# happierpig/flashinfer-ai

Hardware: AMD Instinct MI355X
Metric: paged_decode_hbm_bandwidth_bs64_kv8192_hd128 (higher is better)
Workload: dtype bf16; 1 GPU; C2: BatchDecodeWithPagedKVCacheWrapper bf16 GQA 32/8 head_dim=128 page_size=16 bs=64/GPU kv_len=8192, random page permutation; batch_per_gpu=64, kv_len=8192, num_qo_heads=32, num_kv_heads=8, head_dim=128, page_size=16, split_kv=True, kv_chunk_size=4096, parallelism=batch-shard x1 (no data-path collective)

## Files before the change

### flashinfer-ai_amd/csrc/decode.hip

```cpp
#include <stdlib.h>
#include <string.h>

#include <algorithm>
#include <vector>

#include "decode_kernel.h"
#include "merge_kernel.h"

namespace fi {

#define FI_DECL(DT, HD)                                                                   \
  hipError_t decode_launch_##DT##_##HD(const DecodeKernelParams& p, int gt, int rope, int grid, \
                                       hipStream_t stream);
FI_DECL(0, 64) FI_DECL(0, 128) FI_DECL(0, 256) FI_DECL(0, 512)
FI_DECL(1, 64) FI_DECL(1, 128) FI_DECL(1, 256) FI_DECL(1, 512)
FI_DECL(2, 64) FI_DECL(2, 128) FI_DECL(2, 256) FI_DECL(2, 512)
FI_DECL(3, 64) FI_DECL(3, 128) FI_DECL(3, 256) FI_DECL(3, 512)
#undef FI_DECL

typedef hipError_t (*decode_launch_fn)(const DecodeKernelParams&, int, int, int, hipStream_t);

static decode_launch_fn find_launcher(int kv_dt, int head_dim) {
#define FI_ROW(DT)                          \
  case DT:                                  \
// ... 18 lines not shown
      return nullptr;
  }
#undef FI_ROW
}

static bool decode_mfma16() {
  static const bool on = [] {
    const char* e = getenv("FI_DECODE_MFMA16");
    return !e || atoi(e) != 0;
  }();
  return on;
}

static int decode_waves_per_cu(int kv_dtype, bool batch) {
  const bool fp8 = kv_dtype == FI_DTYPE_FP8_E4M3 || kv_dtype == FI_DTYPE_FP8_E5M2;
  return (batch && !fp8) ? 4 : 8;
}

static int tokens_per_load(int kv_dt, int head_dim) {
  const int vec = 16 / (int)dtype_size(kv_dt);
  return 64 / (head_dim / vec);
}

static int ilog2_exact(int x) {
  if (x <= 0 || (x & (x - 1))) return -1;
  int l = 0;
  while ((1 << l) < x) ++l;
  return l;
}

hipError_t decode_mfma_launch(const DecodeKernelParams& p, int q_dtype, int kv_dtype, int head_dim, int rope, int grid,
                              hipStream_t stream);
hipError_t decode_mfma16_launch(const DecodeKernelParams& p, int q_dtype, int kv_dtype, int head_dim, int rope,
                                int grid, hipStream_t stream);

constexpr int kMfmaMinGroup = 5;
constexpr int kMfmaMinGroupFp8 = 3;

enum class DecodeKernel { VALU, MFMA32, MFMA16 };

struct DecodeChoice {
  DecodeKernel kind;
  int head_tiles;
  int gt;
};

static DecodeChoice choose_decode(int group, int q_dt, int kv_dt, int head_dim, int page_size, bool rope,
                                  bool plain_logits, bool strides_fit_31_bits) {
  DecodeChoice c;
  c.gt = group <= 1 ? 1 : group == 2 ? 2 : 4;
  const bool fp8 = kv_dt == FI_DTYPE_FP8_E4M3 || kv_dt == FI_DTYPE_FP8_E5M2;
  const bool mfma = (q_dt == FI_DTYPE_F16 || q_dt == FI_DTYPE_BF16) && (kv_dt == q_dt || fp8) &&
                    (head_dim == 64 || head_dim == 128) && strides_fit_31_bits;
  if (decode_mfma16()) {
    c.kind = !(mfma && (plain_logits || group <= 16)) ? DecodeKernel::VALU
             : group <= 16                            ? DecodeKernel::MFMA16
                                                      : DecodeKernel::MFMA32;
  } else {
    const bool small_pages = ilog2_exact(page_size) < 0 || page_size < tokens_per_load(kv_dt, head_dim);
    const int min_group = (rope || small_pages) ? 1 : fp8 ? kMfmaMinGroupFp8 : kMfmaMinGroup;
    c.kind = mfma && plain_logits && group >= min_group ? DecodeKernel::MFMA32 : DecodeKernel::VALU;
  }
  c.head_tiles = c.kind == DecodeKernel::VALU ? ceil_div(group, c.gt) : ceil_div(group, 32);
  return c;
}

static int launch_decode(const DecodeKernelParams& kp, const DecodeChoice& c, int q_dt, int kv_dt, int head_dim,
                         bool rope, int merge_n, int merge_rows, hipStream_t stream) {
  if (kp.num_items > 0) {
    const int grid = ceil_div(kp.num_items, kDecodeWaves);
    if (c.kind == DecodeKernel::MFMA16)
      FI_HIP_CALL(decode_mfma16_launch(kp, q_dt, kv_dt, head_dim, rope, grid, stream));
    else if (c.kind == DecodeKernel::MFMA32)
      FI_HIP_CALL(decode_mfma_launch(kp, q_dt, kv_dt, head_dim, rope, grid, stream));
    else
      FI_HIP_CALL(find_launcher(kv_dt, head_dim)(kp, c.gt, rope, grid, stream));
  }
  if (kp.split_kv) {
    MergeNParams mp{kp.tmp_o, kp.tmp_lse, kp.o_indptr, kp.o, kp.lse, merge_n, merge_rows,
                    kp.num_qo_heads, head_dim, FI_DTYPE_F32, q_dt};
    FI_HIP_CALL(launch_merge_n(mp, stream));
  }
  return 0;
}

static int32_t window_pages(const int32_t* indptr_h, int i, int page_size, int window_left) {
  const int32_t np = indptr_h[i + 1] - indptr_h[i];
  if (window_left < 0 || np <= 0) return np;
  const int64_t first = std::max<int64_t>((int64_t)(np - 1) * page_size - window_left, 0) / page_size;
  return (int32_t)(np - first);
}

struct DecodeWork {
  bool split_kv;
  uint32_t pages_per_chunk;
  size_t padded;
};

static DecodeWork estimate_decode_work(const int32_t* indptr_h, int batch_size, int page_size, int window_left,
                                       uint32_t gdy, uint32_t max_grid, bool enable_cuda_graph) {
  std::vector<int32_t> num_pages(batch_size);
  uint32_t max_pages = 0;
  for (int i = 0; i < batch_size; ++i)
    max_pages = std::max<uint32_t>(max_pages, num_pages[i] = window_pages(indptr_h, i, page_size, window_left));
  if ((uint64_t)batch_size * gdy >= max_grid) return {false, std::max(max_pages, 1u), (size_t)batch_size};
// ... 31 lines not shown
  FI_REQUIRE(find_launcher(kv_dtype, head_dim) != nullptr,
             "batch_decode_plan: unsupported kv dtype %d / head_dim %d", kv_dtype, head_dim);
  for (int i = 0; i < batch_size; ++i)
    FI_REQUIRE(indptr_h[i + 1] >= indptr_h[i], "batch_decode_plan: indptr must be non-decreasing");

  const int head_tiles = choose_decode(num_qo_heads / num_kv_heads, q_dtype, kv_dtype, head_dim, page_size,
                                       false, true, true)
                             .head_tiles;
  const uint32_t gdy = (uint32_t)(num_kv_heads * head_tiles);
  const uint32_t max_grid =
      max_grid_hint > 0 ? (uint32_t)max_grid_hint
                        : (uint32_t)(fi_num_compute_units() * decode_waves_per_cu(kv_dtype, true) * (head_tiles > 1 ? 2 : 1));

  if (window_left < 0) window_left = -1;
  const auto [split_kv, pages_per_chunk, padded] =
      estimate_decode_work(indptr_h, batch_size, page_size, window_left, gdy, max_grid, enable_cuda_graph);

  OffsetAllocator ia(int_ws_bytes);
  const int64_t req_off = ia.alloc(padded * sizeof(int32_t));
  const int64_t tile_off = ia.alloc(padded * sizeof(int32_t));
  const int64_t oind_off = ia.alloc(((size_t)batch_size + 1) * sizeof(int32_t));
  const int64_t chunk_off = ia.alloc(sizeof(int32_t));
  int64_t mask_off = 0;
  if (split_kv) mask_off = ia.alloc(padded);
  FI_REQUIRE(ia.ok, "batch_decode_plan: int workspace too small (%zu bytes)", int_ws_bytes);

  char* hp = (char*)pinned_int_ws;
  int32_t* req_h = (int32_t*)(hp + req_off);
  int32_t* tile_h = (int32_t*)(hp + tile_off);
  int32_t* oind_h = (int32_t*)(hp + oind_off);
  memset(req_h, 0, padded * sizeof(int32_t));
  memset(tile_h, 0, padded * sizeof(int32_t));
  size_t w = 0;
  oind_h[0] = 0;
  for (int b = 0; b < batch_size; ++b) {
    const uint32_t np = (uint32_t)std::max(window_pages(indptr_h, b, page_size, window_left), 1);
    const uint32_t nchunks = split_kv ? ceil_div(np, pages_per_chunk) : 1u;
    for (uint32_t t = 0; t < nchunks; ++t) {
      FI_REQUIRE(w < padded, "batch_decode_plan: work list overflow");
      req_h[w] = b;
      tile_h[w] = (int32_t)t;
      ++w;
    }
    oind_h[b + 1] = oind_h[b] + (int32_t)nchunks;
  }
  *(int32_t*)(hp + chunk_off) = (int32_t)(pages_per_chunk * (uint32_t)page_size);
  if (split_kv) {
    uint8_t* mask_h = (uint8_t*)(hp + mask_off);
    for (size_t i = 0; i < padded; ++i) mask_h[i] = i < w;
  }

  int64_t v_off = 0, s_off = 0;
  if (split_kv) {
    OffsetAllocator fa(float_ws_bytes);
    v_off = fa.alloc((size_t)num_qo_heads * padded * head_dim * sizeof(float));
    s_off = fa.alloc((size_t)num_qo_heads * padded * sizeof(float));
    FI_REQUIRE(fa.ok, "batch_decode_plan: float workspace too small (%zu bytes, need %zu)",
               float_ws_bytes, (size_t)num_qo_heads * padded * (head_dim + 1) * sizeof(float));
  }

  for (int i = 0; i < FI_DECODE_PLAN_INFO_LEN; ++i) plan_info_out[i] = 0;
  plan_info_out[FI_DP_PADDED_BATCH_SIZE] = (int64_t)padded;
  plan_info_out[FI_DP_V_OFFSET] = v_off;
  plan_info_out[FI_DP_S_OFFSET] = s_off;
  plan_info_out[FI_DP_REQUEST_INDICES_OFFSET] = req_off;
  plan_info_out[FI_DP_KV_TILE_INDICES_OFFSET] = tile_off;
  plan_info_out[FI_DP_O_INDPTR_OFFSET] = oind_off;
  plan_info_out[FI_DP_BLOCK_VALID_MASK_OFFSET] = mask_off;
  plan_info_out[FI_DP_KV_CHUNK_SIZE_PTR_OFFSET] = chunk_off;
  plan_info_out[FI_DP_ENABLE_CUDA_GRAPH] = enable_cuda_graph ? 1 : 0;
  plan_info_out[FI_DP_SPLIT_KV] = split_kv ? 1 : 0;
  plan_info_out[FI_DP_KV_CHUNK_SIZE] = (int64_t)pages_per_chunk * page_size;
  plan_info_out[FI_DP_NUM_WORK] = (int64_t)w;
  plan_info_out[FI_DP_BATCH_SIZE] = batch_size;
  plan_info_out[FI_DP_INT_BYTES_USED] = (int64_t)ia.used;
  plan_info_out[FI_DP_WINDOW_LEFT] = window_left;
  plan_info_out[FI_DP_MAGIC] = FI_DECODE_PLAN_MAGIC;

  if (int_ws && ia.used)
    FI_HIP_CALL(hipMemcpyAsync(int_ws, pinned_int_ws, ia.used, hipMemcpyHostToDevice,
                               (hipStream_t)stream));
  return 0;
}

namespace fi {

template <class A>
static int check_and_fill_decode(const char* who, const A& a, int kv_dt, int head_dim, int num_kv_heads,
                                 int page_size, int64_t kv_stride_page, int64_t kv_stride_n, int64_t kv_stride_h,
                                 DecodeKernelParams& kp, DecodeChoice& choice) {
  FI_REQUIRE(a.q_dtype == FI_DTYPE_F16 || a.q_dtype == FI_DTYPE_BF16, "%s: q dtype must be f16/bf16", who);
  FI_REQUIRE(num_kv_heads > 0 && a.num_qo_heads % num_kv_heads == 0,
             "%s: num_qo_heads must be a multiple of num_kv_heads", who);
  FI_REQUIRE(find_launcher(kv_dt, head_dim), "%s: unsupported kv dtype %d / head_dim %d", who, kv_dt, head_dim);
  FI_REQUIRE(a.pos_encoding_mode != FI_POS_ALIBI || a.alibi_slopes, "%s: ALIBI needs alibi_slopes", who);
  memset(&kp, 0, sizeof(kp));
  kp.q = a.q;
  kp.o = a.o;
  kp.lse = a.lse;
  kp.alibi_slopes = a.alibi_slopes;
  kp.kv_stride_page = kv_stride_page;
  kp.kv_stride_n = kv_stride_n;
  kp.kv_stride_h = kv_stride_h;
  kp.num_qo_heads = a.num_qo_heads;
  kp.num_kv_heads = num_kv_heads;
  kp.group_size = a.num_qo_heads / num_kv_heads;
  kp.page_size = page_size;
  kp.log2_page_size = ilog2_exact(page_size);
  kp.uniform_page = kp.log2_page_size >= 0 && page_size >= tokens_per_load(kv_dt, head_dim);
  kp.page_div = FastDiv((uint32_t)page_size);
  kp.window_left = a.window_left;
  kp.q_dtype = a.q_dtype;
  kp.use_alibi = a.pos_encoding_mode == FI_POS_ALIBI;
  kp.logits_soft_cap = a.logits_soft_cap > 0.f ? a.logits_soft_cap : 0.f;
  kp.sm_scale = a.sm_scale;
  kp.rope_rcp_scale = a.rope_rcp_scale;
  kp.rope_rcp_theta = a.rope_rcp_theta;
  const bool plain_logits = a.pos_encoding_mode != FI_POS_ALIBI && !(a.logits_soft_cap > 0.f);
  choice = choose_decode(kp.group_size, a.q_dtype, kv_dt, head_dim, page_size,
                         a.pos_encoding_mode == FI_POS_ROPE_LLAMA, plain_logits,
                         kv_stride_page < (1ll << 31) && kv_stride_n < (1ll << 31));
  kp.head_tiles = choice.head_tiles;
  return 0;
}

}

extern "C" FI_API int fi_batch_decode_run(void* float_ws, size_t float_ws_bytes, void* int_ws,
                                   size_t int_ws_bytes, const int64_t* plan_info,
                                   int32_t plan_info_len, const fi_batch_decode_params_t* a,
                                   fi_stream_t stream_) {
  hipStream_t stream = (hipStream_t)stream_;
  FI_REQUIRE(plan_info && plan_info_len == FI_DECODE_PLAN_INFO_LEN &&
                 plan_info[FI_DP_MAGIC] == FI_DECODE_PLAN_MAGIC,
             "batch_decode_run: plan_info is not a decode plan (call plan() first)");
  FI_REQUIRE(a && a->q && a->o && a->kv.k_data && a->kv.v_data && a->kv.indptr &&
                 a->kv.last_page_len,
             "batch_decode_run: null tensor");
  FI_REQUIRE(int_ws, "batch_decode_run: null int workspace");
  const fi_paged_kv_t& kv = a->kv;
  FI_REQUIRE(kv.batch_size == plan_info[FI_DP_BATCH_SIZE],
             "batch_decode_run: batch size %d differs from the planned %lld", kv.batch_size,
             (long long)plan_info[FI_DP_BATCH_SIZE]);
  FI_REQUIRE(a->pos_encoding_mode >= 0 && a->pos_encoding_mode <= 2,
             "batch_decode_run: bad pos_encoding_mode %d", a->pos_encoding_mode);
  DecodeKernelParams kp;
  DecodeChoice choice;
  if (check_and_fill_decode("batch_decode_run", *a, kv.dtype, kv.head_dim, kv.num_kv_heads, kv.page_size,
                            kv.stride_page, kv.stride_n, kv.stride_h, kp, choice))
    return 1;
  const size_t esz = dtype_size(kv.dtype);
  FI_REQUIRE(((uintptr_t)a->q % 16) == 0 && (a->q_stride_n * 2) % 16 == 0 && (a->q_stride_h * 2) % 16 == 0,
             "batch_decode_run: q rows must be 16-byte aligned");
  FI_REQUIRE((kv.stride_n * esz) % 16 == 0 && (kv.stride_h * esz) % 16 == 0 &&
                 (kv.stride_page * esz) % 16 == 0 && ((uintptr_t)kv.k_data % 16) == 0 &&
                 ((uintptr_t)kv.v_data % 16) == 0,
             "batch_decode_run: kv cache rows must be 16-byte aligned");
  if (kv.batch_size == 0) return 0;

  const bool split = plan_info[FI_DP_SPLIT_KV] != 0;
  const int64_t padded = plan_info[FI_DP_PADDED_BATCH_SIZE];
  kp.k = kv.k_data;
  kp.v = kv.v_data;
  kp.indptr = kv.indptr;
  kp.indices = kv.indices;
  kp.last_page_len = kv.last_page_len;
  const char* ib = (const char*)int_ws;
  kp.request_indices = (const int32_t*)(ib + plan_info[FI_DP_REQUEST_INDICES_OFFSET]);
  kp.kv_tile_indices = (const int32_t*)(ib + plan_info[FI_DP_KV_TILE_INDICES_OFFSET]);
  kp.o_indptr = (const int32_t*)(ib + plan_info[FI_DP_O_INDPTR_OFFSET]);
  kp.block_valid_mask =
      (split && plan_info[FI_DP_ENABLE_CUDA_GRAPH])
          ? (const uint8_t*)(ib + plan_info[FI_DP_BLOCK_VALID_MASK_OFFSET])
          : nullptr;
  (void)int_ws_bytes;
  kp.q_rope_offset = a->q_rope_offset;
  kp.kv_rope_pos_offset = kv.rope_pos_offset;
  kp.q_stride_n = a->q_stride_n;
  kp.q_stride_h = a->q_stride_h;
  kp.num_items = (int32_t)(padded * kv.num_kv_heads * kp.head_tiles);
  kp.kv_chunk_size = (int32_t)plan_info[FI_DP_KV_CHUNK_SIZE];
  kp.kv_chunk_size_ptr = (const int32_t*)(ib + plan_info[FI_DP_KV_CHUNK_SIZE_PTR_OFFSET]);
  kp.split_kv = split;
  kp.plan_window_left = (int32_t)plan_info[FI_DP_WINDOW_LEFT];
  FI_REQUIRE(kp.plan_window_left < 0 || kp.plan_window_left == a->window_left,
             "batch_decode_run: window_left %d differs from the planned %d", a->window_left, kp.plan_window_left);
  if (split) {
    FI_REQUIRE(float_ws, "batch_decode_run: split-kv plan needs the float workspace");
    const size_t need = (size_t)plan_info[FI_DP_S_OFFSET] +
                        (size_t)a->num_qo_heads * padded * sizeof(float);
    FI_REQUIRE(need <= float_ws_bytes, "batch_decode_run: float workspace too small");
    kp.tmp_o = (float*)((char*)float_ws + plan_info[FI_DP_V_OFFSET]);
    kp.tmp_lse = (float*)((char*)float_ws + plan_info[FI_DP_S_OFFSET]);
  }
  kp.fast_path = kp.uniform_page && kp.indices && !kp.use_alibi && kp.logits_soft_cap == 0.f;
  return launch_decode(kp, choice, a->q_dtype, kv.dtype, kv.head_dim, a->pos_encoding_mode == FI_POS_ROPE_LLAMA,
                       0, kv.batch_size, stream);
}

extern "C" FI_API int fi_single_decode_run(const fi_single_decode_params_t* a, void* tmp, size_t tmp_bytes,
                                    fi_stream_t stream_) {
  hipStream_t stream = (hipStream_t)stream_;
  FI_REQUIRE(a && a->q && a->k && a->v && a->o, "single_decode_run: null tensor");
  FI_REQUIRE(a->kv_len >= 0, "single_decode_run: negative kv_len");
  const int vpage = 16;
  DecodeKernelParams kp;
  DecodeChoice choice;
  if (check_and_fill_decode("single_decode_run", *a, a->kv_dtype, a->head_dim, a->num_kv_heads, vpage,
                            (int64_t)vpage * a->kv_stride_n, a->kv_stride_n, a->kv_stride_h, kp, choice))
    return 1;
  const size_t esz = dtype_size(a->kv_dtype);
  FI_REQUIRE(((uintptr_t)a->q % 16) == 0 && (a->q_stride_h * 2) % 16 == 0,
             "single_decode_run: q rows must be 16-byte aligned");
  FI_REQUIRE((a->kv_stride_n * esz) % 16 == 0 && (a->kv_stride_h * esz) % 16 == 0 &&
                 ((uintptr_t)a->k % 16) == 0 && ((uintptr_t)a->v % 16) == 0,
             "single_decode_run: k/v rows must be 16-byte aligned");

  kp.k = a->k;
  kp.v = a->v;
  kp.q_stride_n = 0;
  kp.q_stride_h = a->q_stride_h;
  kp.single_kv_len = a->kv_len;
  kp.plan_window_left = -1;
  const int gdy = a->num_kv_heads * kp.head_tiles;
  const int max_grid = fi_num_compute_units() * decode_waves_per_cu(a->kv_dtype, false);
  int chunk = a->kv_len, nchunks = 1;
  if (a->kv_len > 256 && tmp) {
    const int want = std::max(1, max_grid / gdy);
    chunk = std::max(ceil_div(a->kv_len, want), 256);
    chunk = ceil_div(chunk, vpage) * vpage;
    nchunks = ceil_div(a->kv_len, chunk);
    const size_t need = (size_t)nchunks * a->num_qo_heads * (a->head_dim + 1) * sizeof(float) + 64;
    if (need > tmp_bytes || nchunks <= 1) {
      chunk = a->kv_len;
      nchunks = 1;
    }
  }
  kp.split_kv = nchunks > 1;
  kp.kv_chunk_size = chunk;
  kp.num_items = nchunks * gdy;
  if (kp.split_kv) {
    kp.tmp_o = (float*)tmp;
    size_t vbytes = (size_t)nchunks * a->num_qo_heads * a->head_dim * sizeof(float);
    vbytes = (vbytes + 15) / 16 * 16;
    kp.tmp_lse = (float*)((char*)tmp + vbytes);
  }
  return launch_decode(kp, choice, a->q_dtype, a->kv_dtype, a->head_dim, a->pos_encoding_mode == FI_POS_ROPE_LLAMA,
                       nchunks, 1, stream);
}
```

### flashinfer-ai_amd/csrc/decode_mfma16_inst.hip

```cpp
#include "decode_mfma16_kernel.h"

namespace fi {

template <int T16, int KVS, int D>
static hipError_t launch16(const DecodeKernelParams& p, int rope, int grid, hipStream_t stream) {
  const dim3 g(grid), b(kDecodeThreads);
  if (rope) {
    if (p.indices) decode_mfma16_kernel<T16, KVS, D, true, true><<<g, b, 0, stream>>>(p);
    else decode_mfma16_kernel<T16, KVS, D, false, true><<<g, b, 0, stream>>>(p);
  } else {
    if (p.indices) decode_mfma16_kernel<T16, KVS, D, true, false><<<g, b, 0, stream>>>(p);
    else decode_mfma16_kernel<T16, KVS, D, false, false><<<g, b, 0, stream>>>(p);
  }
  return hipGetLastError();
}

hipError_t decode_mfma16_launch(const DecodeKernelParams& p, int q_dtype, int kv_dtype, int head_dim, int rope,
                                int grid, hipStream_t stream) {
#define FI_CASE(T, K, D) \
  if (q_dtype == T && kv_dtype == K && head_dim == D) return launch16<T, K, D>(p, rope, grid, stream);
#define FI_ROW(T, K) FI_CASE(T, K, 64) FI_CASE(T, K, 128)
  FI_ROW(FI_DTYPE_F16, FI_DTYPE_F16)
  FI_ROW(FI_DTYPE_F16, FI_DTYPE_FP8_E4M3)
  FI_ROW(FI_DTYPE_F16, FI_DTYPE_FP8_E5M2)
  FI_ROW(FI_DTYPE_BF16, FI_DTYPE_BF16)
  FI_ROW(FI_DTYPE_BF16, FI_DTYPE_FP8_E4M3)
  FI_ROW(FI_DTYPE_BF16, FI_DTYPE_FP8_E5M2)
#undef FI_ROW
#undef FI_CASE
  return hipErrorInvalidValue;
}

}
```

### flashinfer-ai_amd/csrc/decode_mfma16_kernel.h

```cpp
#pragma once
#include "decode_kernel.h"
#include "prefill_kernel.h"

namespace fi {

template <int T16>
struct Mfma16;
template <>
struct Mfma16<FI_DTYPE_F16> {
  static __device__ __forceinline__ f32x4 mfma(MfmaType<FI_DTYPE_F16>::frag a, MfmaType<FI_DTYPE_F16>::frag b, f32x4 c) {
    return __builtin_amdgcn_mfma_f32_16x16x32_f16(a, b, c, 0, 0, 0);
  }
};
template <>
struct Mfma16<FI_DTYPE_BF16> {
  static __device__ __forceinline__ f32x4 mfma(MfmaType<FI_DTYPE_BF16>::frag a, MfmaType<FI_DTYPE_BF16>::frag b, f32x4 c) {
    return __builtin_amdgcn_mfma_f32_16x16x32_bf16(a, b, c, 0, 0, 0);
  }
};

template <bool MAX>
__device__ __forceinline__ float reduce_rows(float x) {
  const uint32_t u = __builtin_bit_cast(uint32_t, x);
  const auto r = __builtin_amdgcn_permlane16_swap(u, u, false, false);
  const uint32_t r0 = r[0], r1 = r[1];
  const float a = __builtin_bit_cast(float, r0), b = __builtin_bit_cast(float, r1);
  const float y = MAX ? fmaxf(a, b) : a + b;
  const uint32_t v = __builtin_bit_cast(uint32_t, y);
  const auto q = __builtin_amdgcn_permlane32_swap(v, v, false, false);
  const uint32_t q0 = q[0], q1 = q[1];
  const float c = __builtin_bit_cast(float, q0), d = __builtin_bit_cast(float, q1);
  return MAX ? fmaxf(c, d) : c + d;
}

template <int T16, int KVS, int D, bool PAGED, bool ROPE>
__global__ void __launch_bounds__(kDecodeThreads, (ROPE && D == 128 && KVS != T16) ? 1 : 2)
    decode_mfma16_kernel(const DecodeKernelParams p) {
  using M = MfmaType<T16>;
  using frag_t = typename M::frag;
  constexpr int kTile = 32;
  constexpr bool KV_FP8 = (KVS == FI_DTYPE_FP8_E4M3 || KVS == FI_DTYPE_FP8_E5M2);
  constexpr int KV_BYTES = KV_FP8 ? 1 : 2;
  constexpr int ROWB = D * 2;
  constexpr int CPR = D / 8;
  constexpr int GCH = D * KV_BYTES / 16;
  constexpr int RPP = 64 / GCH;
  constexpr int NPASS = kTile / RPP;
  constexpr int KSTEPS = D / 32;
  constexpr int DBLK = D / 16;
  constexpr int TILE_BYTES = kTile * ROWB;
  constexpr int NE = KV_FP8 ? 16 : 8;
  static_assert(D == 64 || D == 128, "head_dim 64 / 128");

  __shared__ __attribute__((aligned(16))) char smem[kDecodeWaves][2 * TILE_BYTES];
  __shared__ __attribute__((aligned(16))) float rope_step[ROPE ? GCH * NE * 2 : 4];

  const int lane = threadIdx.x & 63;
  const int wave = __builtin_amdgcn_readfirstlane((int)(threadIdx.x >> 6));
  int lb;
  {
    const int b = blockIdx.x, total = gridDim.x;
    const int xcd = b & 7, slot = b >> 3;
    const int qn = total >> 3, rn = total & 7;
    lb = (xcd < rn ? xcd * (qn + 1) : rn * (qn + 1) + (xcd - rn) * qn) + slot;
  }
  const int item = lb * kDecodeWaves + wave;
  if (item >= p.num_items) return;
  char* const kb = smem[wave];
  char* const vb = kb + TILE_BYTES;
  const int lc = lane & 15, lg = lane >> 4;

  const int kv_head = item % p.num_kv_heads;
  const int work = item / p.num_kv_heads;
  int req = 0, kv_tile = work;
  if (p.request_indices) {
    if (p.block_valid_mask && !p.block_valid_mask[work]) return;
    req = p.request_indices[work];
    kv_tile = p.kv_tile_indices[work];
  }
  int page_begin = 0, kv_len;
  if (p.indptr) {
    page_begin = p.indptr[req];
    const int np = p.indptr[req + 1] - page_begin;
    kv_len = np > 0 ? (np - 1) * p.page_size + p.last_page_len[req] : 0;
  } else {
    kv_len = p.single_kv_len;
  }
  int chunk_base = 0;
  if (p.plan_window_left >= 0 && p.indptr) {
    const int np = p.indptr[req + 1] - page_begin;
    chunk_base = np > 0 ? max((np - 1) * p.page_size - p.plan_window_left, 0) / p.page_size * p.page_size : 0;
  }
  const int win_start = p.window_left >= 0 ? max(0, kv_len - 1 - p.window_left) : 0;
  const int kv_chunk_size = p.kv_chunk_size_ptr ? *p.kv_chunk_size_ptr : p.kv_chunk_size;
  int chunk_start = chunk_base + (p.split_kv ? kv_tile * kv_chunk_size : 0);
  const int chunk_end = p.split_kv ? min(chunk_start + kv_chunk_size, kv_len) : kv_len;
  if (win_start > chunk_start) chunk_start += (win_start - chunk_start) / kTile * kTile;
  const int G = p.group_size;
  const int head0 = kv_head * G;
  const int head = head0 + min(lc, G - 1);

  frag_t qf[KSTEPS];
  {
    const uint16_t* qrow = (const uint16_t*)p.q + (int64_t)req * p.q_stride_n + (int64_t)head * p.q_stride_h;
#pragma unroll
    for (int ks = 0; ks < KSTEPS; ++ks)
      qf[ks] = __builtin_bit_cast(frag_t, *(const u32x4*)(qrow + 32 * ks + 8 * lg));
    if constexpr (ROPE) {
      const int q_pos = p.q_rope_offset ? p.q_rope_offset[req] : (kv_len - 1);
#pragma unroll
      for (int ks = 0; ks < KSTEPS / 2; ++ks) {
        const u32x4 lo4 = __builtin_bit_cast(u32x4, qf[ks]), hi4 = __builtin_bit_cast(u32x4, qf[ks + KSTEPS / 2]);
        u32x4 out_lo, out_hi;
#pragma unroll
        for (int w = 0; w < 4; ++w) {
          const uint32_t lo_w = lo4[w], hi_w = hi4[w];
          float ra[2], rb[2];
#pragma unroll
          for (int e = 0; e < 2; ++e) {
            const int i = 32 * ks + 8 * lg + 2 * w + e;
            const float freq = p.rope_rcp_scale * __powf(p.rope_rcp_theta, (float)(2 * i) / (float)D);
            float sn, cs;
            sincos_ool((float)q_pos * freq, &sn, &cs);
            const float a = M::to_f32((uint16_t)(lo_w >> (16 * e)));
            const float b = M::to_f32((uint16_t)(hi_w >> (16 * e)));
            ra[e] = a * cs - b * sn;
            rb[e] = b * cs + a * sn;
          }
          out_lo[w] = pack2<T16>(ra[0], ra[1]);
// ... 220 lines not shown
      for (int h = 0; h < 2; ++h)
#pragma unroll
        for (int j2 = 0; j2 < 2; ++j2) {
          const float a = s_acc[h][2 * j2], b = s_acc[h][2 * j2 + 1];
          const uint32_t pk = pack2<T16>(a, b);
          w[2 * h + j2] = pk;
          if constexpr (T16 == FI_DTYPE_BF16) {
            const float ha = __builtin_bit_cast(float, pk << 16);
            const float hb = __builtin_bit_cast(float, pk & 0xffff0000u);
            wl[2 * h + j2] = pack2<T16>(a - ha, b - hb);
          }
        }
      const frag_t pfrag = __builtin_bit_cast(frag_t, w);
#pragma unroll
      for (int db = 0; db < DBLK; ++db) {
        const char* base = vb + v_rd[db];
        const s16x4 lo = __builtin_amdgcn_ds_read_tr16_b64_v4i16((__attribute__((address_space(3))) s16x4*)(base));
        const s16x4 hi = __builtin_amdgcn_ds_read_tr16_b64_v4i16(
            (__attribute__((address_space(3))) s16x4*)(base + 16 * ROWB));
        using s16x8 = __attribute__((ext_vector_type(8))) short;
        const s16x8 a8 = {lo[0], lo[1], lo[2], lo[3], hi[0], hi[1], hi[2], hi[3]};
        o_acc[db] = Mfma16<T16>::mfma(__builtin_bit_cast(frag_t, a8), pfrag, o_acc[db]);
        if constexpr (T16 == FI_DTYPE_BF16)
          o_acc[db] = Mfma16<T16>::mfma(__builtin_bit_cast(frag_t, a8), __builtin_bit_cast(frag_t, wl), o_acc[db]);
      }
      __builtin_amdgcn_wave_barrier();
    }
  }

  l_run = reduce_rows<false>(l_run);
  const bool empty = !(l_run > 0.f);
  const float inv = empty ? 0.f : 1.0f / l_run;
  const float lse_v = empty ? FI_NEG_INF : m_run + fast_log2(l_run);
  if (lc < G) {
    const int qo_head = head0 + lc;
    const int64_t out_row = p.split_kv ? (int64_t)(p.o_indptr ? p.o_indptr[req] : 0) + kv_tile : req;
    const int64_t ob = (out_row * p.num_qo_heads + qo_head) * D;
#pragma unroll
    for (int db = 0; db < DBLK; ++db) {
      const int d0 = 16 * db + 4 * lg;
      if (p.split_kv) {
        *(f32x4*)(p.tmp_o + ob + d0) = o_acc[db] * inv;
      } else {
        const uint32_t w0 = pack2<T16>(o_acc[db][0] * inv, o_acc[db][1] * inv);
        const uint32_t w1 = pack2<T16>(o_acc[db][2] * inv, o_acc[db][3] * inv);
        *(u32x2*)((uint16_t*)p.o + ob + d0) = u32x2{w0, w1};
      }
    }
    if (lg == 0) {
      if (p.split_kv) p.tmp_lse[out_row * p.num_qo_heads + qo_head] = lse_v;
      else if (p.lse) p.lse[out_row * p.num_qo_heads + qo_head] = lse_v;
    }
  }
}

}
```

### flashinfer-ai_amd/flashinfer/_lib.py

```python
from __future__ import annotations

import ctypes as C
import os
from typing import Optional

import torch

_HERE = os.path.dirname(os.path.abspath(__file__))
_LIB_PATH = os.environ.get("FI_MI355_LIB", os.path.join(_HERE, "libfi_mi355.so"))

FI_DTYPE_F16, FI_DTYPE_BF16, FI_DTYPE_FP8_E4M3, FI_DTYPE_FP8_E5M2, FI_DTYPE_F32 = range(5)
FI_NEG_INF = -5.0e4
FI_DECODE_PLAN_INFO_LEN = 16

_TORCH2FI = {
    torch.float16: FI_DTYPE_F16,
    torch.bfloat16: FI_DTYPE_BF16,
    torch.float8_e4m3fn: FI_DTYPE_FP8_E4M3,
    torch.float8_e5m2: FI_DTYPE_FP8_E5M2,
    torch.float32: FI_DTYPE_F32,
}


def fi_dtype(dtype: torch.dtype) -> int:
    try:
        return _TORCH2FI[dtype]
    except KeyError:
        raise ValueError(f"unsupported dtype {dtype} for the MI355X kernels") from None


class PagedKV(C.Structure):
    _fields_ = [
        ("k_data", C.c_void_p),
        ("v_data", C.c_void_p),
        ("indptr", C.c_void_p),
        ("indices", C.c_void_p),
        ("last_page_len", C.c_void_p),
        ("rope_pos_offset", C.c_void_p),
        ("stride_page", C.c_int64),
        ("stride_n", C.c_int64),
        ("stride_h", C.c_int64),
        ("page_size", C.c_int32),
        ("num_kv_heads", C.c_int32),
        ("head_dim", C.c_int32),
        ("batch_size", C.c_int32),
        ("dtype", C.c_int32),
# ... 212 lines not shown
    _fields_ = [
        ("in_", C.c_void_p), ("out", C.c_void_p), ("top_k_arr", C.c_void_p), ("scalar_arr", C.c_void_p),
        ("top_k_val", C.c_int32), ("scalar_val", C.c_float),
        ("batch", C.c_int32), ("vocab", C.c_int32), ("param_len", C.c_int32),
    ]


class ChainSpeculativeParams(C.Structure):
    _fields_ = [
        ("draft_probs", C.c_void_p), ("draft_token_ids", C.c_void_p), ("target_probs", C.c_void_p),
        ("output_token_ids", C.c_void_p), ("output_accepted_token_num", C.c_void_p),
        ("output_emitted_draft_token_num", C.c_void_p),
        ("batch", C.c_int32), ("num_speculative_tokens", C.c_int32), ("vocab", C.c_int32),
        ("philox_seed", C.c_uint64), ("philox_offset", C.c_uint64),
    ]


FI_PREFILL_PLAN_INFO_LEN = 16
FI_PREFILL_PLAN_MAGIC = 0x4649505245
FI_PREFILL_QKVO_PLAN_MAGIC = 0x4649514B564F
FI_MLA_PLAN_INFO_LEN = 16
(FI_MLA_NUM_WORK, FI_MLA_GRID, FI_MLA_TOTAL_ROWS, FI_MLA_KV_CHUNK_SIZE, FI_MLA_SPLIT_KV, FI_MLA_ENABLE_CUDA_GRAPH,
 FI_MLA_NUM_HEADS, FI_MLA_BATCH_SIZE, FI_MLA_INT_BYTES_USED, FI_MLA_MERGE_INDPTR_OFFSET, FI_MLA_ITEMS_OFFSET,
 FI_MLA_NUM_ENTRIES, FI_MLA_V_OFFSET, FI_MLA_PAGE_SIZE, FI_MLA_DTYPE, FI_MLA_MAGIC) = range(16)

_lib: Optional[C.CDLL] = None

EXPORTED_SYMBOLS = [
    "fi_last_error",
    "fi_abi_version",
    "fi_num_compute_units",
    "fi_batch_decode_plan",
    "fi_batch_decode_run",
    "fi_single_decode_run",
    "fi_merge_state",
    "fi_merge_state_in_place",
    "fi_merge_states",
    "fi_variable_length_merge_states",
    "fi_batch_prefill_plan",
    "fi_batch_prefill_paged_run",
    "fi_single_prefill_run",
    "fi_batch_prefill_qkvo_run",
    "fi_single_prefill_qkvo_run",
    "fi_gemm_fp8_nt_groupwise",
    "fi_group_gemm_fp8_nt_groupwise",
    "fi_get_batch_indices_positions",
    "fi_append_paged_kv_cache",
    "fi_apply_rope_pos_ids",
    "fi_apply_rope_append_paged_kv_cache",
    "fi_rope_positions_from_indptr",
    "fi_packbits",
    "fi_segment_packbits",
    "fi_batch_mla_plan",
    "fi_batch_mla_run",
    "fi_append_paged_mla_kv_cache",
    "fi_softmax",
    "fi_sampling_from_logits",
    "fi_sampling_from_probs",
    "fi_top_k_sampling_from_probs",
    "fi_top_p_sampling_from_probs",
    "fi_min_p_sampling_from_probs",
    "fi_top_k_top_p_sampling_from_probs",
    "fi_top_p_renorm_probs",
    "fi_top_k_renorm_probs",
    "fi_top_k_mask_logits",
    "fi_chain_speculative_sampling",
]

SAMPLING_SYMBOLS = ("fi_sampling_from_logits", "fi_sampling_from_probs", "fi_top_k_sampling_from_probs",
                    "fi_top_p_sampling_from_probs", "fi_min_p_sampling_from_probs",
                    "fi_top_k_top_p_sampling_from_probs")
ROW_TRANSFORM_SYMBOLS = ("fi_softmax", "fi_top_p_renorm_probs", "fi_top_k_renorm_probs", "fi_top_k_mask_logits")


def lib() -> C.CDLL:
    global _lib
    if _lib is not None:
        return _lib
    if not os.path.exists(_LIB_PATH):
        raise RuntimeError(
            f"{_LIB_PATH} not found: build it with `make -C flashinfer-ai_amd/csrc -j8` "
            "(or python -c 'import __graft_entry__ as g; g.build()').  There is no CPU fallback."
        )
    l = C.CDLL(_LIB_PATH)
    l.fi_last_error.restype = C.c_char_p
    l.fi_abi_version.restype = C.c_int
    l.fi_num_compute_units.restype = C.c_int
    vp, i32, i64p, sz = C.c_void_p, C.c_int32, C.POINTER(C.c_int64), C.c_size_t
    l.fi_batch_decode_plan.argtypes = [vp, sz, vp, vp, sz, vp, i32, i32, i32, i32, i32, i32, i32, i32, i32, i32, i64p, vp]
    l.fi_batch_decode_run.argtypes = [vp, sz, vp, sz, i64p, i32, C.POINTER(BatchDecodeParams), vp]
    l.fi_single_decode_run.argtypes = [C.POINTER(SingleDecodeParams), vp, sz, vp]
    l.fi_merge_state.argtypes = [vp, vp, vp, vp, vp, vp, i32, i32, i32, i32, vp]
    l.fi_merge_state_in_place.argtypes = [vp, vp, vp, vp, vp, i32, i32, i32, i32, vp]
    l.fi_merge_states.argtypes = [vp, vp, vp, vp, i32, i32, i32, i32, i32, vp]
    l.fi_variable_length_merge_states.argtypes = [vp, vp, vp, vp, vp, i32, i32, i32, i32, i32, vp]
    l.fi_batch_prefill_plan.argtypes = [vp, sz, vp, vp, sz, vp, vp, vp] + [i32] * 12 + [i64p, vp]
    l.fi_batch_prefill_paged_run.argtypes = [vp, sz, vp, sz, i64p, i32, C.POINTER(BatchPrefillParams), vp]
    l.fi_single_prefill_run.argtypes = [C.POINTER(SinglePrefillParams), vp, sz, vp]
    l.fi_batch_prefill_qkvo_run.argtypes = [vp, sz, vp, sz, i64p, i32, C.POINTER(PrefillQkvoParams), vp]
    l.fi_single_prefill_qkvo_run.argtypes = [C.POINTER(PrefillQkvoParams), vp, sz, vp]
    l.fi_gemm_fp8_nt_groupwise.argtypes = [vp] * 5 + [i32] * 10 + [vp]
    l.fi_group_gemm_fp8_nt_groupwise.argtypes = [vp] * 6 + [i32] * 11 + [vp]
    l.fi_packbits.argtypes = [vp, C.c_int64, i32, vp, vp]
    l.fi_segment_packbits.argtypes = [vp, vp, vp, i32, C.c_int64, i32, vp, vp]
    l.fi_get_batch_indices_positions.argtypes = [vp, vp, i32, i32, vp, vp, vp]
    l.fi_append_paged_kv_cache.argtypes = [vp, vp, C.c_int64, C.c_int64, C.c_int64, C.c_int64, vp, vp, i32, C.POINTER(PagedKV), vp]
    l.fi_apply_rope_pos_ids.argtypes = [C.POINTER(RopeParams), vp]
    l.fi_apply_rope_append_paged_kv_cache.argtypes = [C.POINTER(RopeParams), vp, C.c_int64, C.c_int64, vp, vp, C.POINTER(PagedKV), vp]
    l.fi_rope_positions_from_indptr.argtypes = [vp, vp, i32, i32, vp, vp]
    l.fi_batch_mla_plan.argtypes = [C.POINTER(MlaPlanParams), i64p, vp]
    l.fi_batch_mla_run.argtypes = [i64p, i32, C.POINTER(MlaParams), vp]
    l.fi_append_paged_mla_kv_cache.argtypes = [C.POINTER(AppendMlaParams), vp]
    for name in SAMPLING_SYMBOLS:
        getattr(l, name).argtypes = [C.POINTER(SamplingParams), vp]
    for name in ROW_TRANSFORM_SYMBOLS:
        getattr(l, name).argtypes = [C.POINTER(RowTransformParams), vp]
    l.fi_chain_speculative_sampling.argtypes = [C.POINTER(ChainSpeculativeParams), vp]
    for name in EXPORTED_SYMBOLS:
        fn = getattr(l, name)
        if name not in ("fi_last_error",):
            fn.restype = C.c_int
    _lib = l
    return l
# ... 60 lines not shown
```

### include/fi_mi355.h

```cpp
#ifndef FI_MI355_H_
#define FI_MI355_H_

#include <stddef.h>
#include <stdint.h>

#ifdef __cplusplus
extern "C" {
#endif

#define FI_ABI_VERSION 2
#define FI_NEG_INF (-5.0e4f)

typedef void* fi_stream_t;

#if defined(FI_BUILDING_LIB)
#define FI_API __attribute__((visibility("default")))
#else
#define FI_API
#endif

enum fi_dtype {
  FI_DTYPE_F16 = 0,
  FI_DTYPE_BF16 = 1,
  FI_DTYPE_FP8_E4M3 = 2,
  FI_DTYPE_FP8_E5M2 = 3,
  FI_DTYPE_F32 = 4
};

enum fi_pos_encoding_mode { FI_POS_NONE = 0, FI_POS_ROPE_LLAMA = 1, FI_POS_ALIBI = 2 };
enum fi_mask_mode { FI_MASK_NON_CAUSAL = 0, FI_MASK_CAUSAL = 1, FI_MASK_CUSTOM = 2, FI_MASK_MULTIITEMSCORING = 3 };

FI_API const char* fi_last_error(void);
FI_API int fi_abi_version(void);
FI_API int fi_num_compute_units(void);

typedef struct fi_paged_kv {
  const void* k_data;
  const void* v_data;
  const int32_t* indptr;
  const int32_t* indices;
  const int32_t* last_page_len;
  const int32_t* rope_pos_offset;
  int64_t stride_page, stride_n, stride_h;
  int32_t page_size;
  int32_t num_kv_heads;
  int32_t head_dim;
  int32_t batch_size;
  int32_t dtype;
} fi_paged_kv_t;

#define FI_DECODE_PLAN_INFO_LEN 16
enum fi_decode_plan_slot {
  FI_DP_PADDED_BATCH_SIZE = 0,
  FI_DP_V_OFFSET = 1,
  FI_DP_S_OFFSET = 2,
  FI_DP_REQUEST_INDICES_OFFSET = 3,
  FI_DP_KV_TILE_INDICES_OFFSET = 4,
  FI_DP_O_INDPTR_OFFSET = 5,
  FI_DP_BLOCK_VALID_MASK_OFFSET = 6,
  FI_DP_KV_CHUNK_SIZE_PTR_OFFSET = 7,
  FI_DP_ENABLE_CUDA_GRAPH = 8,
  FI_DP_SPLIT_KV = 9,
  FI_DP_KV_CHUNK_SIZE = 10,
  FI_DP_NUM_WORK = 11,
  FI_DP_BATCH_SIZE = 12,
  FI_DP_INT_BYTES_USED = 13,
  FI_DP_WINDOW_LEFT = 14,
  FI_DP_MAGIC = 15
};
#define FI_DECODE_PLAN_MAGIC 0x4649444543ll

FI_API int fi_batch_decode_plan(void* float_ws, size_t float_ws_bytes, void* int_ws, void* pinned_int_ws,
                         size_t int_ws_bytes, const int32_t* indptr_h, int32_t batch_size,
                         int32_t num_qo_heads, int32_t num_kv_heads, int32_t page_size,
                         int32_t enable_cuda_graph, int32_t head_dim, int32_t q_dtype,
                         int32_t kv_dtype, int32_t max_grid_hint, int32_t window_left,
                         int64_t* plan_info_out, fi_stream_t stream);

typedef struct fi_batch_decode_params {
  const void* q;
  int64_t q_stride_n, q_stride_h;
  fi_paged_kv_t kv;
  void* o;
  float* lse;
  const float* alibi_slopes;
  const int32_t* q_rope_offset;
  int32_t num_qo_heads;
  int32_t q_dtype;
  int32_t pos_encoding_mode;
  int32_t window_left;
  float logits_soft_cap;
  float sm_scale;
  float rope_rcp_scale;
  float rope_rcp_theta;
} fi_batch_decode_params_t;

FI_API int fi_batch_decode_run(void* float_ws, size_t float_ws_bytes, void* int_ws, size_t int_ws_bytes,
                        const int64_t* plan_info, int32_t plan_info_len,
                        const fi_batch_decode_params_t* params, fi_stream_t stream);

typedef struct fi_single_decode_params {
  const void* q;
  int64_t q_stride_h;
  const void* k;
  const void* v;
  int64_t kv_stride_n, kv_stride_h;
  void* o;
  float* lse;
  const float* alibi_slopes;
  int32_t kv_len, num_qo_heads, num_kv_heads, head_dim;
  int32_t q_dtype, kv_dtype;
  int32_t pos_encoding_mode;
  int32_t window_left;
  float logits_soft_cap, sm_scale, rope_rcp_scale, rope_rcp_theta;
} fi_single_decode_params_t;

FI_API int fi_single_decode_run(const fi_single_decode_params_t* params, void* tmp, size_t tmp_bytes,
                         fi_stream_t stream);

FI_API int fi_merge_state(const void* v_a, const float* s_a, const void* v_b, const float* s_b,
                   void* v_merged, float* s_merged, int32_t seq_len, int32_t num_heads,
                   int32_t head_dim, int32_t dtype, fi_stream_t stream);
FI_API int fi_merge_state_in_place(void* v, float* s, const void* v_other, const float* s_other,
                            const uint8_t* mask, int32_t seq_len, int32_t num_heads,
                            int32_t head_dim, int32_t dtype, fi_stream_t stream);
FI_API int fi_merge_states(const void* v, const float* s, void* v_merged, float* s_merged,
                    int32_t num_index_sets, int32_t seq_len, int32_t num_heads, int32_t head_dim,
                    int32_t dtype, fi_stream_t stream);
FI_API int fi_variable_length_merge_states(const void* v, const float* s, const int32_t* indptr,
                                    void* v_merged, float* s_merged, int32_t seq_len,
                                    int32_t num_heads, int32_t head_dim, int32_t in_dtype,
                                    int32_t out_dtype, fi_stream_t stream);
// ... 293 lines not shown
```

Measured before the change: 6651 GB/s.

## Fold split-KV chunks into one workgroup and merge in LDS, dropping merge kernel

When a paged MFMA16 split-KV decode has at most four chunks per request, the waves of one workgroup each process a chunk of the same request and KV head. The partial outputs and LSEs go through shared memory and are combined by the chunk-0 wave, which writes the final output directly. This removes the separate merge launch and the round trip of the fp32 tmp_o/tmp_lse buffers through HBM. In exchange, fewer KV heads are handled per workgroup, a workgroup-wide barrier is added, and the plan info gains a max_chunks slot, which changes the ABI length.

```diff
diff --git a/flashinfer-ai_amd/csrc/decode.hip b/flashinfer-ai_amd/csrc/decode.hip
--- a/flashinfer-ai_amd/csrc/decode.hip
+++ b/flashinfer-ai_amd/csrc/decode.hip
@@ -74,7 +74,7 @@
 hipError_t decode_mfma_launch(const DecodeKernelParams& p, int q_dtype, int kv_dtype, int head_dim, int rope, int grid,
                               hipStream_t stream);
 hipError_t decode_mfma16_launch(const DecodeKernelParams& p, int q_dtype, int kv_dtype, int head_dim, int rope,
-                                int grid, hipStream_t stream);
+                                int nc, int grid, hipStream_t stream);
 
 constexpr int kMfmaMinGroup = 5;
 constexpr int kMfmaMinGroupFp8 = 3;
@@ -107,12 +107,24 @@
   return c;
 }
 
+static int decode_fold_chunks(const DecodeChoice& c, bool split_kv, bool graph_plan, int64_t max_chunks, bool rope,
+                              bool paged) {
+  if (!split_kv || graph_plan || c.kind != DecodeKernel::MFMA16 || rope || !paged) return 0;
+  if (max_chunks < 1 || max_chunks > 4) return 0;
+  return max_chunks <= 2 ? 2 : 4;
+}
+
 static int launch_decode(const DecodeKernelParams& kp, const DecodeChoice& c, int q_dt, int kv_dt, int head_dim,
-                         bool rope, int merge_n, int merge_rows, hipStream_t stream) {
+                         bool rope, int merge_n, int merge_rows, int fold_nc, hipStream_t stream) {
+  if (fold_nc) {
+    const int grid = merge_rows * ceil_div(kp.num_kv_heads, kDecodeWaves / fold_nc);
+    FI_HIP_CALL(decode_mfma16_launch(kp, q_dt, kv_dt, head_dim, rope, fold_nc, grid, stream));
+    return 0;
+  }
   if (kp.num_items > 0) {
     const int grid = ceil_div(kp.num_items, kDecodeWaves);
     if (c.kind == DecodeKernel::MFMA16)
-      FI_HIP_CALL(decode_mfma16_launch(kp, q_dt, kv_dt, head_dim, rope, grid, stream));
+      FI_HIP_CALL(decode_mfma16_launch(kp, q_dt, kv_dt, head_dim, rope, 0, grid, stream));
     else if (c.kind == DecodeKernel::MFMA32)
       FI_HIP_CALL(decode_mfma_launch(kp, q_dt, kv_dt, head_dim, rope, grid, stream));
     else
@@ -210,6 +222,7 @@
   memset(req_h, 0, padded * sizeof(int32_t));
   memset(tile_h, 0, padded * sizeof(int32_t));
   size_t w = 0;
+  uint32_t max_chunks = 0;
   oind_h[0] = 0;
   for (int b = 0; b < batch_size; ++b) {
     const uint32_t np = (uint32_t)std::max(window_pages(indptr_h, b, page_size, window_left), 1);
@@ -221,6 +234,7 @@
       ++w;
     }
     oind_h[b + 1] = oind_h[b] + (int32_t)nchunks;
+    max_chunks = std::max(max_chunks, nchunks);
   }
   *(int32_t*)(hp + chunk_off) = (int32_t)(pages_per_chunk * (uint32_t)page_size);
   if (split_kv) {
@@ -254,6 +268,7 @@
   plan_info_out[FI_DP_INT_BYTES_USED] = (int64_t)ia.used;
   plan_info_out[FI_DP_WINDOW_LEFT] = window_left;
   plan_info_out[FI_DP_MAGIC] = FI_DECODE_PLAN_MAGIC;
+  plan_info_out[FI_DP_MAX_CHUNKS] = max_chunks;
 
   if (int_ws && ia.used)
     FI_HIP_CALL(hipMemcpyAsync(int_ws, pinned_int_ws, ia.used, hipMemcpyHostToDevice,
@@ -304,6 +319,36 @@
 
 }
 
+static int batch_decode_launches(const int64_t* plan_info, int32_t plan_info_len, const fi_batch_decode_params_t* a,
+                                 DecodeKernelParams& kp, DecodeChoice& choice, int& fold_nc) {
+  fold_nc = 0;
+  if (!(plan_info && plan_info_len == FI_DECODE_PLAN_INFO_LEN && plan_info[FI_DP_MAGIC] == FI_DECODE_PLAN_MAGIC)) {
+    set_error("batch_decode: plan_info is not a decode plan (call plan() first)");
+    return -1;
+  }
+  if (!a) {
+    set_error("batch_decode: null params");
+    return -1;
+  }
+  const fi_paged_kv_t& kv = a->kv;
+  if (check_and_fill_decode("batch_decode", *a, kv.dtype, kv.head_dim, kv.num_kv_heads, kv.page_size, kv.stride_page,
+                            kv.stride_n, kv.stride_h, kp, choice))
+    return -1;
+  if (kv.batch_size == 0) return 0;
+  const bool split = plan_info[FI_DP_SPLIT_KV] != 0;
+  fold_nc = decode_fold_chunks(choice, split, plan_info[FI_DP_ENABLE_CUDA_GRAPH] != 0, plan_info[FI_DP_MAX_CHUNKS],
+                               a->pos_encoding_mode == FI_POS_ROPE_LLAMA, kv.indices != nullptr);
+  return split && !fold_nc ? 2 : 1;
+}
+
+extern "C" FI_API int fi_batch_decode_num_launches(const int64_t* plan_info, int32_t plan_info_len,
+                                            const fi_batch_decode_params_t* a) {
+  DecodeKernelParams kp;
+  DecodeChoice choice;
+  int fold_nc;
+  return batch_decode_launches(plan_info, plan_info_len, a, kp, choice, fold_nc);
+}
+
 extern "C" FI_API int fi_batch_decode_run(void* float_ws, size_t float_ws_bytes, void* int_ws,
                                    size_t int_ws_bytes, const int64_t* plan_info,
                                    int32_t plan_info_len, const fi_batch_decode_params_t* a,
@@ -324,9 +369,8 @@
              "batch_decode_run: bad pos_encoding_mode %d", a->pos_encoding_mode);
   DecodeKernelParams kp;
   DecodeChoice choice;
-  if (check_and_fill_decode("batch_decode_run", *a, kv.dtype, kv.head_dim, kv.num_kv_heads, kv.page_size,
-                            kv.stride_page, kv.stride_n, kv.stride_h, kp, choice))
-    return 1;
+  int fold_nc;
+  if (batch_decode_launches(plan_info, plan_info_len, a, kp, choice, fold_nc) < 0) return 1;
   const size_t esz = dtype_size(kv.dtype);
   FI_REQUIRE(((uintptr_t)a->q % 16) == 0 && (a->q_stride_n * 2) % 16 == 0 && (a->q_stride_h * 2) % 16 == 0,
              "batch_decode_run: q rows must be 16-byte aligned");
@@ -373,7 +417,7 @@
   }
   kp.fast_path = kp.uniform_page && kp.indices && !kp.use_alibi && kp.logits_soft_cap == 0.f;
   return launch_decode(kp, choice, a->q_dtype, kv.dtype, kv.head_dim, a->pos_encoding_mode == FI_POS_ROPE_LLAMA,
-                       0, kv.batch_size, stream);
+                       0, kv.batch_size, fold_nc, stream);
 }
 
 extern "C" FI_API int fi_single_decode_run(const fi_single_decode_params_t* a, void* tmp, size_t tmp_bytes,
@@ -424,5 +468,5 @@
     kp.tmp_lse = (float*)((char*)tmp + vbytes);
   }
   return launch_decode(kp, choice, a->q_dtype, a->kv_dtype, a->head_dim, a->pos_encoding_mode == FI_POS_ROPE_LLAMA,
-                       nchunks, 1, stream);
-}
+                       nchunks, 1, 0, stream);
+}
diff --git a/flashinfer-ai_amd/csrc/decode_mfma16_fused_inst.hip b/flashinfer-ai_amd/csrc/decode_mfma16_fused_inst.hip
--- /dev/null
+++ b/flashinfer-ai_amd/csrc/decode_mfma16_fused_inst.hip
@@ -0,0 +1,31 @@
+#include "decode_mfma16_kernel.h"
+
+namespace fi {
+
+template <int T16, int KVS, int D>
+static hipError_t launch16_fused(const DecodeKernelParams& p, int nc, int grid, hipStream_t stream) {
+  const dim3 g(grid), b(kDecodeThreads);
+  if (nc == 2) decode_mfma16_kernel<T16, KVS, D, true, false, 2><<<g, b, 0, stream>>>(p);
+  else if (nc == 4) decode_mfma16_kernel<T16, KVS, D, true, false, 4><<<g, b, 0, stream>>>(p);
+  else return hipErrorInvalidValue;
+  return hipGetLastError();
+}
+
+hipError_t decode_mfma16_fused_launch(const DecodeKernelParams& p, int q_dtype, int kv_dtype, int head_dim, int nc,
+                                      int grid, hipStream_t stream) {
+  if (!p.indices || !p.o_indptr || !p.split_kv) return hipErrorInvalidValue;
+#define FI_CASE(T, K, D) \
+  if (q_dtype == T && kv_dtype == K && head_dim == D) return launch16_fused<T, K, D>(p, nc, grid, stream);
+#define FI_ROW(T, K) FI_CASE(T, K, 64) FI_CASE(T, K, 128)
+  FI_ROW(FI_DTYPE_F16, FI_DTYPE_F16)
+  FI_ROW(FI_DTYPE_F16, FI_DTYPE_FP8_E4M3)
+  FI_ROW(FI_DTYPE_F16, FI_DTYPE_FP8_E5M2)
+  FI_ROW(FI_DTYPE_BF16, FI_DTYPE_BF16)
+  FI_ROW(FI_DTYPE_BF16, FI_DTYPE_FP8_E4M3)
+  FI_ROW(FI_DTYPE_BF16, FI_DTYPE_FP8_E5M2)
+#undef FI_ROW
+#undef FI_CASE
+  return hipErrorInvalidValue;
+}
+
+}
diff --git a/flashinfer-ai_amd/csrc/decode_mfma16_inst.hip b/flashinfer-ai_amd/csrc/decode_mfma16_inst.hip
--- a/flashinfer-ai_amd/csrc/decode_mfma16_inst.hip
+++ b/flashinfer-ai_amd/csrc/decode_mfma16_inst.hip
@@ -15,8 +15,12 @@
   return hipGetLastError();
 }
 
+hipError_t decode_mfma16_fused_launch(const DecodeKernelParams& p, int q_dtype, int kv_dtype, int head_dim, int nc,
+                                      int grid, hipStream_t stream);
+
 hipError_t decode_mfma16_launch(const DecodeKernelParams& p, int q_dtype, int kv_dtype, int head_dim, int rope,
-                                int grid, hipStream_t stream) {
+                                int nc, int grid, hipStream_t stream) {
+  if (nc) return decode_mfma16_fused_launch(p, q_dtype, kv_dtype, head_dim, nc, grid, stream);
 #define FI_CASE(T, K, D) \
   if (q_dtype == T && kv_dtype == K && head_dim == D) return launch16<T, K, D>(p, rope, grid, stream);
 #define FI_ROW(T, K) FI_CASE(T, K, 64) FI_CASE(T, K, 128)
diff --git a/flashinfer-ai_amd/csrc/decode_mfma16_kernel.h b/flashinfer-ai_amd/csrc/decode_mfma16_kernel.h
--- a/flashinfer-ai_amd/csrc/decode_mfma16_kernel.h
+++ b/flashinfer-ai_amd/csrc/decode_mfma16_kernel.h
@@ -1,4 +1,6 @@
 #pragma once
+#include <type_traits>
+
 #include "decode_kernel.h"
 #include "prefill_kernel.h"
 
@@ -33,7 +35,7 @@
   return MAX ? fmaxf(c, d) : c + d;
 }
 
-template <int T16, int KVS, int D, bool PAGED, bool ROPE>
+template <int T16, int KVS, int D, bool PAGED, bool ROPE, int NC = 0>
 __global__ void __launch_bounds__(kDecodeThreads, (ROPE && D == 128 && KVS != T16) ? 1 : 2)
     decode_mfma16_kernel(const DecodeKernelParams p) {
   using M = MfmaType<T16>;
@@ -51,6 +53,8 @@
   constexpr int TILE_BYTES = kTile * ROWB;
   constexpr int NE = KV_FP8 ? 16 : 8;
   static_assert(D == 64 || D == 128, "head_dim 64 / 128");
+  static_assert(NC == 0 || ((NC == 2 || NC == 4) && !ROPE), "chunks folded per workgroup: 2 or 4, without fused RoPE");
+  static_assert(DBLK * 64 * 16 + 64 * 4 <= 2 * TILE_BYTES, "partial state larger than the K | V region");
 
   __shared__ __attribute__((aligned(16))) char smem[kDecodeWaves][2 * TILE_BYTES];
   __shared__ __attribute__((aligned(16))) float rope_step[ROPE ? GCH * NE * 2 : 4];
@@ -64,19 +68,33 @@
     const int qn = total >> 3, rn = total & 7;
     lb = (xcd < rn ? xcd * (qn + 1) : rn * (qn + 1) + (xcd - rn) * qn) + slot;
   }
-  const int item = lb * kDecodeWaves + wave;
-  if (item >= p.num_items) return;
   char* const kb = smem[wave];
   char* const vb = kb + TILE_BYTES;
   const int lc = lane & 15, lg = lane >> 4;
 
-  const int kv_head = item % p.num_kv_heads;
-  const int work = item / p.num_kv_heads;
-  int req = 0, kv_tile = work;
-  if (p.request_indices) {
-    if (p.block_valid_mask && !p.block_valid_mask[work]) return;
-    req = p.request_indices[work];
-    kv_tile = p.kv_tile_indices[work];
+  int kv_head, req = 0, kv_tile;
+  [[maybe_unused]] int n_chunks = 1;
+  [[maybe_unused]] bool active = true;
+  if constexpr (NC > 0) {
+    constexpr int HPW = kDecodeWaves / NC;
+    const int hgroups = (p.num_kv_heads + HPW - 1) / HPW;
+    req = lb / hgroups;
+    kv_head = (lb - req * hgroups) * HPW + wave / NC;
+    kv_tile = wave % NC;
+    n_chunks = p.o_indptr[req + 1] - p.o_indptr[req];
+    active = kv_head < p.num_kv_heads && kv_tile < n_chunks;
+    kv_head = min(kv_head, p.num_kv_heads - 1);
+  } else {
+    const int item = lb * kDecodeWaves + wave;
+    if (item >= p.num_items) return;
+    kv_head = item % p.num_kv_heads;
+    const int work = item / p.num_kv_heads;
+    kv_tile = work;
+    if (p.request_indices) {
+      if (p.block_valid_mask && !p.block_valid_mask[work]) return;
+      req = p.request_indices[work];
+      kv_tile = p.kv_tile_indices[work];
+    }
   }
   int page_begin = 0, kv_len;
   if (p.indptr) {
@@ -94,7 +112,9 @@
   const int win_start = p.window_left >= 0 ? max(0, kv_len - 1 - p.window_left) : 0;
   const int kv_chunk_size = p.kv_chunk_size_ptr ? *p.kv_chunk_size_ptr : p.kv_chunk_size;
   int chunk_start = chunk_base + (p.split_kv ? kv_tile * kv_chunk_size : 0);
-  const int chunk_end = p.split_kv ? min(chunk_start + kv_chunk_size, kv_len) : kv_len;
+  int chunk_end = p.split_kv ? min(chunk_start + kv_chunk_size, kv_len) : kv_len;
+  if constexpr (NC > 0)
+    if (!active) chunk_end = chunk_start;
   if (win_start > chunk_start) chunk_start += (win_start - chunk_start) / kTile * kTile;
   const int G = p.group_size;
   const int head0 = kv_head * G;
@@ -381,6 +401,64 @@
   const bool empty = !(l_run > 0.f);
   const float inv = empty ? 0.f : 1.0f / l_run;
   const float lse_v = empty ? FI_NEG_INF : m_run + fast_log2(l_run);
+  if constexpr (NC > 0) {
+    constexpr int LSE_OFF = DBLK * 64 * 4;
+    if (active && kv_tile > 0) {
+      float* const mine = (float*)smem[wave];
+#pragma unroll
+      for (int db = 0; db < DBLK; ++db) *(f32x4*)(mine + (db * 64 + lane) * 4) = o_acc[db] * inv;
+      mine[LSE_OFF + lane] = lse_v;
+    }
+    __syncthreads();
+    if (active && kv_tile == 0) {
+      auto fold = [&](auto full) {
+#pragma clang fp contract(off)
+        constexpr bool FULL = decltype(full)::value;
+        float s[4] = {lse_v, 0.f, 0.f, 0.f}, w[4];
+#pragma unroll
+        for (int j = 1; j < NC; ++j)
+          if (FULL || j < n_chunks) s[j] = ((const float*)smem[wave + j])[LSE_OFF + lane];
+        float mx = -1.0e30f;
+#pragma unroll
+        for (int j = 0; j < NC; ++j)
+          if (FULL || j < n_chunks) mx = fmaxf(mx, s[j]);
+#pragma unroll
+        for (int j = 0; j < 4; ++j) w[j] = (j < NC && (FULL || j < n_chunks)) ? fast_exp2(s[j] - mx) : 0.f;
+        const float dsum = (w[0] + w[2]) + (w[1] + w[3]);
+        const bool none = !(dsum > 0.f) || mx <= FI_NEG_INF;
+        const float inv_d = none ? 0.f : 1.0f / dsum;
+        if (lc < G) {
+          const int qo_head = head0 + lc;
+          const int64_t ob = ((int64_t)req * p.num_qo_heads + qo_head) * D;
+#pragma unroll
+          for (int db = 0; db < DBLK; ++db) {
+            const f32x4 v0 = o_acc[db] * inv;
+            f32x4 acc;
+#pragma unroll
+            for (int i = 0; i < 4; ++i) acc[i] = __builtin_fmaf(w[0], v0[i], 0.f);
+#pragma unroll
+            for (int j = 1; j < 4; ++j) {
+              f32x4 e = {0.f, 0.f, 0.f, 0.f};
+              if (j < NC && (FULL || j < n_chunks)) {
+                const f32x4 vj = *(const f32x4*)((const float*)smem[wave + j] + (db * 64 + lane) * 4);
+#pragma unroll
+                for (int i = 0; i < 4; ++i) e[i] = __builtin_fmaf(w[j], vj[i], 0.f);
+              }
+              acc = acc + e;
+            }
+            const uint32_t w0 = pack2<T16>(acc[0] * inv_d, acc[1] * inv_d);
+            const uint32_t w1 = pack2<T16>(acc[2] * inv_d, acc[3] * inv_d);
+            *(u32x2*)((uint16_t*)p.o + ob + 16 * db + 4 * lg) = u32x2{w0, w1};
+          }
+          if (lg == 0 && p.lse)
+            p.lse[(int64_t)req * p.num_qo_heads + qo_head] = none ? FI_NEG_INF : mx + fast_log2(dsum);
+        }
+      };
+      if (n_chunks == NC) fold(std::true_type{});
+      else fold(std::false_type{});
+    }
+    return;
+  }
   if (lc < G) {
     const int qo_head = head0 + lc;
     const int64_t out_row = p.split_kv ? (int64_t)(p.o_indptr ? p.o_indptr[req] : 0) + kv_tile : req;
diff --git a/flashinfer-ai_amd/flashinfer/_lib.py b/flashinfer-ai_amd/flashinfer/_lib.py
--- a/flashinfer-ai_amd/flashinfer/_lib.py
+++ b/flashinfer-ai_amd/flashinfer/_lib.py
@@ -11,7 +11,7 @@
 
 FI_DTYPE_F16, FI_DTYPE_BF16, FI_DTYPE_FP8_E4M3, FI_DTYPE_FP8_E5M2, FI_DTYPE_F32 = range(5)
 FI_NEG_INF = -5.0e4
-FI_DECODE_PLAN_INFO_LEN = 16
+FI_DECODE_PLAN_INFO_LEN = 17
 
 _TORCH2FI = {
     torch.float16: FI_DTYPE_F16,
@@ -290,6 +290,7 @@
     "fi_num_compute_units",
     "fi_batch_decode_plan",
     "fi_batch_decode_run",
+    "fi_batch_decode_num_launches",
     "fi_single_decode_run",
     "fi_merge_state",
     "fi_merge_state_in_place",
@@ -347,6 +348,7 @@
     vp, i32, i64p, sz = C.c_void_p, C.c_int32, C.POINTER(C.c_int64), C.c_size_t
     l.fi_batch_decode_plan.argtypes = [vp, sz, vp, vp, sz, vp, i32, i32, i32, i32, i32, i32, i32, i32, i32, i32, i64p, vp]
     l.fi_batch_decode_run.argtypes = [vp, sz, vp, sz, i64p, i32, C.POINTER(BatchDecodeParams), vp]
+    l.fi_batch_decode_num_launches.argtypes = [i64p, i32, C.POINTER(BatchDecodeParams)]
     l.fi_single_decode_run.argtypes = [C.POINTER(SingleDecodeParams), vp, sz, vp]
     l.fi_merge_state.argtypes = [vp, vp, vp, vp, vp, vp, i32, i32, i32, i32, vp]
     l.fi_merge_state_in_place.argtypes = [vp, vp, vp, vp, vp, i32, i32, i32, i32, vp]
diff --git a/include/fi_mi355.h b/include/fi_mi355.h
--- a/include/fi_mi355.h
+++ b/include/fi_mi355.h
@@ -49,7 +49,7 @@
   int32_t dtype;
 } fi_paged_kv_t;
 
-#define FI_DECODE_PLAN_INFO_LEN 16
+#define FI_DECODE_PLAN_INFO_LEN 17
 enum fi_decode_plan_slot {
   FI_DP_PADDED_BATCH_SIZE = 0,
   FI_DP_V_OFFSET = 1,
@@ -66,7 +66,8 @@
   FI_DP_BATCH_SIZE = 12,
   FI_DP_INT_BYTES_USED = 13,
   FI_DP_WINDOW_LEFT = 14,
-  FI_DP_MAGIC = 15
+  FI_DP_MAGIC = 15,
+  FI_DP_MAX_CHUNKS = 16
 };
 #define FI_DECODE_PLAN_MAGIC 0x4649444543ll
 
@@ -98,6 +99,9 @@
 FI_API int fi_batch_decode_run(void* float_ws, size_t float_ws_bytes, void* int_ws, size_t int_ws_bytes,
                         const int64_t* plan_info, int32_t plan_info_len,
                         const fi_batch_decode_params_t* params, fi_stream_t stream);
+
+FI_API int fi_batch_decode_num_launches(const int64_t* plan_info, int32_t plan_info_len,
+                                 const fi_batch_decode_params_t* params);
 
 typedef struct fi_single_decode_params {
   const void* q;
```

After: 6653 GB/s (median of 5 runs). About the same (+0.0%).
